# Layjins/Spider

Hardware: AMD Instinct MI355X
Metric: multimodal responses/sec (text->text+image) (higher is better)
Workload: dtype bf16

## Files before the change

### include/spider_hip.h

```cpp
#ifndef SPIDER_HIP_H
#define SPIDER_HIP_H
#define SPIDER_ABI_VERSION 4

#ifdef __cplusplus
extern "C" {
#endif

int spider_abi_version(void);
const char* spider_target_arch(void);
const char* spider_last_error(void);


int spider_embed_bf16(const void* table, const int* ids, void* out, int rows, int H, int V, void* stream);

int spider_rmsnorm_bf16(const void* x, const void* res, const void* w, void* y, void* res_out, int rows, int H,
                        float eps, void* stream);

int spider_gemv_bf16(const void* W, const void* x, void* out, const void* bias, const void* res, const void* norm_w,
                     float eps, int B, int N, int K, void* stream);

int spider_gemv_swiglu_bf16(const void* W_gate_up, const void* x, void* out, const void* norm_w, float eps, int B,
                            int I, int K, void* stream);

int spider_lm_head_nparts(int V);

int spider_decode_advance_i32(const int* next_ids, int* cur_ids, int* pos, int* slot, int* kv_end, int* hist, int* n_hist,
                              int cap, int B, void* stream);
int spider_lm_head_argmax_bf16(const void* W, const void* x, const void* norm_w, float eps, int* out_ids, void* logits,
                               void* ws_val, void* ws_idx, int B, int V, int K, void* stream);

int spider_lm_head_argmax_proc_bf16(const void* W, const void* x, const void* norm_w, float eps, int* out_ids, void* logits,
                                    void* ws_val, void* ws_idx, const void* seen, const void* ban, const float* penalty,
                                    const int* min_new, const int* eos_ids, const int* n_eos, const int* n_hist, int B, int V,
                                    int K, void* stream);
int spider_decode_advance_seen_i32(const int* next_ids, int* cur_ids, int* pos, int* slot, int* kv_end, int* hist, int* n_hist,
                                   void* seen, int V, int cap, int B, void* stream);
int spider_token_bitmap_set_i32(const int* ids, void* bitmap, int B, int n, int V, void* stream);

int spider_beam_partial_bf16(const void* logits, float* ws_ms, float* ws_val, int* ws_tok, int rows, int V, int C, int nslice,
                             void* stream);
int spider_beam_select_f32(const float* ws_ms, const float* ws_val, const int* ws_tok, float* run_scores, const int* eos_ids,
                           const int* n_eos, const int* n_hist, float* trace_score, int* trace_beam, int* trace_tok, int cap,
                           int* src_beam, int* next_ids, int B, int K, int V, int C, int nslice, void* stream);
int spider_kv_row_gather_bf16(void* k_cache, void* v_cache, void* k_tmp, void* v_tmp, const int* src_beam, const int* kv_beg,
                              const int* kv_end, int K, int R, int layers, int rows_alloc, int n_kv, int T, int d, void* stream);

int spider_rope_kv_append_bf16(const void* qkv, const int* pos, const int* slot, const float* cos_sin, void* q_out,
                               void* k_cache, void* v_cache, int B, int S, int n_q, int n_kv, int d, int T_max,
                               void* stream);
int spider_rope_kv_append_mrope_bf16(const void* qkv, const int* pos3, const int* slot, const float* cos_sin, void* q_out,
                                     void* k_cache, void* v_cache, int B, int S, int n_q, int n_kv, int d, int T_max,
                                     int sec_t, int sec_h, void* stream);

int spider_attn_decode_bf16(const void* q, const void* k_cache, const void* v_cache, const int* kv_beg,
                            const int* kv_end, void* out, void* ws_o, void* ws_ml, int B, int n_q, int n_kv, int d,
                            int T_max, float scale, int nsplit, void* stream);

int spider_attn_decode_fused_bf16(const void* qkv, const int* pos, const float* cos_sin, void* k_cache, void* v_cache,
                                  const int* kv_beg, const int* kv_end, void* out, void* ws_o, void* ws_ml,
                                  int* counters, int B, int n_q, int n_kv, int d, int T_max, float scale, int nsplit,
                                  void* stream);
int spider_set_attn_inline(int on);
int spider_set_ws_inlaunch(int on);

int spider_gemv_fm_bf16(const void* Wfm, const void* x, void* out, const void* bias, const void* res, int B, int N, int K,
                        int fold_rmsnorm, float eps, void* stream);
int spider_gemv_swiglu_fm_bf16(const void* Wfm_gate_up, const void* x, void* out, int B, int I, int K, int fold_rmsnorm, float eps,
                               void* stream);
int spider_lm_head_argmax_fm_bf16(const void* Wfm, const void* x, int* out_ids, void* logits, void* ws_val, void* ws_idx, int B,
                                  int V, int K, int fold_rmsnorm, float eps, void* stream);
int spider_lm_head_argmax_fm_proc_bf16(const void* Wfm, const void* x, int* out_ids, void* logits, void* ws_val, void* ws_idx,
                                       const void* seen, const void* ban, const float* penalty, const int* min_new,
                                       const int* eos_ids, const int* n_eos, const int* n_hist, int B, int V, int K,
                                       int fold_rmsnorm, float eps, void* stream);


int spider_gemm_bf16(const void* A, const void* W, void* C, void* C32, const void* bias, const void* res,
                     const void* rowbias, int rows_per_group, int M, int N, int K, int lda, int ldc, int act,
                     float out_scale, int w_tiled, const float* res32, float* c32d, void* ws, long ws_bytes, void* stream);

int spider_gemm_ln_bf16(const void* A, const void* Wf, void* C, const float* colsum, const float* colbias, const void* res,
                        int M, int N, int K, int ldc, int act, float eps, int w_tiled, void* ws, long ws_bytes, void* stream);

int spider_xattn_fused_bf16(const void* x, const void* mq_fm, const void* mo_fm, const float* colsum, const float* colbias,
                            const void* bias_o, void* out, int B2, int n_tok, int C, int heads, int n_keys, float eps,
                            const float* x32, float* out32, void* stream);

int spider_conv2d_nhwc_bf16(const void* x, const void* w, void* y, const void* bias, const void* res,
                            const void* rowbias, int B, int Hin, int Win, int Cin, int Cout, int ks, int stride,
                            int pad, int ups, float out_scale, int w_tiled, const float* res32, float* c32d, void* ws, long ws_bytes, void* stream);

int spider_conv_nhwc_ex_bf16(const void* x, const void* w, void* y, const void* bias, const void* res,
                             const void* rowbias, int B, int Hin, int Win, int Cin, int Cout, int kh, int kw, int stride,
                             int pad_h, int pad_w, int dil, int up_h, int up_w, int act, float act_param,
                             float out_scale, int w_tiled, const float* res32, float* c32d, void* ws, long ws_bytes, void* stream);

int spider_attn_bf16(const void* q, const void* k, const void* v, void* o,
                     long q_bs, long q_hs, long q_rs, long k_bs, long k_hs, long k_rs,
                     long v_bs, long v_hs, long v_rs, long o_bs, long o_hs, long o_rs,
                     int B, int Hq, int Hkv, int Lq, int Lk, int d, float scale, int causal, int kv_off,
                     const int* kv_beg, const void* keep_bits, int blk, int q_off, void* stream);

int spider_story_key_lists_i32(const void* keep_bits, int n_keys, int N, int img0, int n_lists, int q_img0, int stride,
                               int* key_idx, int* tiles, void* stream);
int spider_attn_keylist_bf16(const void* q, const void* k, const void* v, void* o,
                             long q_bs, long q_hs, long q_rs, long k_bs, long k_hs, long k_rs,
                             long v_bs, long v_hs, long v_rs, long o_bs, long o_hs, long o_rs,
                             int B, int Hq, int Hkv, int Lq, int Lk, int d, float scale,
                             const int* key_idx, int idx_len, const int* tiles, int n_tiles, void* stream);

int spider_attn_varlen_bf16(const void* q, const void* k, const void* v, void* o, long q_rs, long k_rs, long v_rs, long o_rs,
                            int total_rows, int Hq, int Hkv, int d, float scale, const int* tiles, int n_tiles, void* stream);

int spider_rope_rows_bf16(void* x, const float* cos_sin, long row_stride, int rows, int heads, int d, void* stream);


int spider_groupnorm_nchunk(int HW);
int spider_groupnorm_nhwc_bf16(const void* x, const void* gamma, const void* beta, void* y, void* ws, int B, int HW,
                               int C, int G, float eps, int silu, void* stream);
int spider_groupnorm_cat_nhwc_bf16(const void* x1, const void* x2, const void* gamma, const void* beta, void* y, void* cat,
                                   void* ws, int B, int HW, int C1, int C2, int G, float eps, int silu, void* stream);
int spider_conv_nhwc_gn_bf16(const void* x, const void* w, void* y, const void* bias, const void* res, const void* rowbias,
                             int B, int Hin, int Win, int Cin, int Cout, int kh, int kw, int stride, int pad_h, int pad_w,
                             int dil, int up_h, int up_w, int act, float act_param, float out_scale, int w_tiled,
                             const float* res32, float* c32d, void* ws, long ws_bytes, void* stream,
                             float* gn_part, int gn_groups, int* produced);
int spider_groupnorm_stats_nhwc_bf16(const void* x, void* partial, int B, int HW, int C, int G, int nchunk, void* stream);
int spider_groupnorm_apply_nhwc_bf16(const void* x, const void* partial, int nchunk, const void* gamma, const void* beta, void* y,
                                     int B, int HW, int C, int G, float eps, int silu, void* stream);
int spider_gemm_gn_in_bf16(const void* A, const void* W, void* C, const void* bias, int M, int N, int K, int ldc, int w_tiled,
                           const float* gn_part, int nchunk, const void* gamma, const void* beta, int G, float eps, int HW,
                           float* c32d, void* stream);
int spider_layernorm_bf16(const void* x, const void* gamma, const void* beta, void* y, int rows, int C, float eps,
                          void* stream);
int spider_geglu_bf16(const void* x, void* y, int M, int inner, void* stream);
int spider_swiglu_bf16(const void* x, void* y, int M, int inner, void* stream);
int spider_concat_channels_bf16(const void* a, const void* b, void* y, long rows, int C1, int C2, void* stream);
int spider_act_bf16(const void* x, void* y, long n, int act, void* stream);
int spider_add_bf16(const void* a, const void* b, void* y, long n, void* stream);
int spider_act_ex_bf16(const void* x, void* y, long n, int act, float param, void* stream);
int spider_add_scaled_bf16(const void* a, const void* b, void* y, long n, float scale, void* stream);
int spider_axpby_bf16(const void* a, const void* b, void* y, long n, float alpha, float beta, void* stream);
int spider_mean_tokens_bf16(const void* x, void* y, int B, int T, int C, void* stream);
int spider_moe_combine_bf16(const void* const* host_xs, int E, const void* logits, int ld, void* y, int B, long per_batch,
                            void* stream);
// ... 132 lines not shown
```

### spider_amd/csrc/llm_decode.hip

```cpp
#include "common.hpp"
#include <stdlib.h>

using namespace spider;

__global__ __launch_bounds__(256) void embed_kernel(const bf16_t* __restrict__ table, const int* __restrict__ ids,
                                                    bf16_t* __restrict__ out, int H, int V) {
    const int r = blockIdx.x;
    int id = ids[r];
    id = id < 0 ? 0 : (id >= V ? V - 1 : id);
    const u32x4* src = reinterpret_cast<const u32x4*>(table + (size_t)id * H);
    u32x4* dst = reinterpret_cast<u32x4*>(out + (size_t)r * H);
    for (int i = threadIdx.x; i < H / 8; i += 256) dst[i] = src[i];
}

__global__ __launch_bounds__(256) void rope_rows_kernel(bf16_t* __restrict__ x, const float* __restrict__ cs, long row_stride,
                                                        int rows, int heads, int d) {
    const int half = d >> 1, cpr = half >> 3;
    const long total = (long)rows * heads * cpr;
    for (long idx = (long)blockIdx.x * 256 + threadIdx.x; idx < total; idx += (long)gridDim.x * 256) {
        const int c = (int)(idx % cpr);
        const int h = (int)((idx / cpr) % heads);
        const long r = idx / ((long)cpr * heads);
        bf16_t* p = x + r * row_stride + (long)h * d + c * 8;
        const u32x4 lo = *reinterpret_cast<const u32x4*>(p);
// ... 13 lines not shown
            float r0 = b0 * co[2 * j], r1 = a0 * si[2 * j], r2 = b1 * co[2 * j + 1], r3 = a1 * si[2 * j + 1];
            asm volatile("" : "+v"(p0), "+v"(p1), "+v"(p2), "+v"(p3), "+v"(r0), "+v"(r1), "+v"(r2), "+v"(r3));
            ol[j] = pack_bf16x2(p0 - p1, p2 - p3);
            oh[j] = pack_bf16x2(r0 + r1, r2 + r3);
        }
        u32x4 vl, vh;
        vl.x = ol[0]; vl.y = ol[1]; vl.z = ol[2]; vl.w = ol[3];
        vh.x = oh[0]; vh.y = oh[1]; vh.z = oh[2]; vh.w = oh[3];
        *reinterpret_cast<u32x4*>(p) = vl;
        *reinterpret_cast<u32x4*>(p + half) = vh;
    }
}

__global__ __launch_bounds__(256) void rmsnorm_kernel(const bf16_t* __restrict__ x, const bf16_t* __restrict__ res,
                                                      const bf16_t* __restrict__ w, bf16_t* __restrict__ y,
                                                      bf16_t* __restrict__ res_out, int H, float eps) {
    __shared__ float red[4];
    const size_t row = blockIdx.x;
    const u32x4* xv = reinterpret_cast<const u32x4*>(x + row * H);
    const u32x4* rv = res ? reinterpret_cast<const u32x4*>(res + row * H) : nullptr;
    const u32x4* wv = reinterpret_cast<const u32x4*>(w);
    u32x4* yv = reinterpret_cast<u32x4*>(y + row * H);
    u32x4* rov = res_out ? reinterpret_cast<u32x4*>(res_out + row * H) : nullptr;
    const int nv = H / 8;
    float h[4][8];
    float ss = 0.f;
#pragma unroll
    for (int it = 0; it < 4; ++it) {
        const int i = threadIdx.x + it * 256;
        if (i < nv) {
            u32x4 a = xv[i];
            uint32_t aw[4] = {a.x, a.y, a.z, a.w};
            if (rv) {
                u32x4 b = rv[i];
                uint32_t bw[4] = {b.x, b.y, b.z, b.w};
#pragma unroll
                for (int j = 0; j < 4; ++j) {
                    float lo = bf16_to_f32(f32_to_bf16(bf16lo_to_f32(aw[j]) + bf16lo_to_f32(bw[j])));
                    float hi = bf16_to_f32(f32_to_bf16(bf16hi_to_f32(aw[j]) + bf16hi_to_f32(bw[j])));
                    h[it][2 * j] = lo;
                    h[it][2 * j + 1] = hi;
                }
                if (rov) {
                    u32x4 o;
                    o.x = pack_bf16x2(h[it][0], h[it][1]);
                    o.y = pack_bf16x2(h[it][2], h[it][3]);
                    o.z = pack_bf16x2(h[it][4], h[it][5]);
                    o.w = pack_bf16x2(h[it][6], h[it][7]);
                    rov[i] = o;
                }
            } else {
#pragma unroll
                for (int j = 0; j < 4; ++j) {
                    h[it][2 * j] = bf16lo_to_f32(aw[j]);
                    h[it][2 * j + 1] = bf16hi_to_f32(aw[j]);
                }
            }
#pragma unroll
            for (int j = 0; j < 8; ++j) ss += h[it][j] * h[it][j];
        }
    }
    const float tot = block_sum<4>(ss, red);
    const float rs = rsqrtf(tot / (float)H + eps);
#pragma unroll
    for (int it = 0; it < 4; ++it) {
        const int i = threadIdx.x + it * 256;
        if (i < nv) {
            u32x4 wq = wv[i];
            uint32_t ww[4] = {wq.x, wq.y, wq.z, wq.w};
            uint32_t o[4];
#pragma unroll
            for (int j = 0; j < 4; ++j) {
                float lo = bf16_to_f32(f32_to_bf16(h[it][2 * j] * rs)) * bf16lo_to_f32(ww[j]);
                float hi = bf16_to_f32(f32_to_bf16(h[it][2 * j + 1] * rs)) * bf16hi_to_f32(ww[j]);
                o[j] = pack_bf16x2(lo, hi);
            }
            u32x4 ov;
            ov.x = o[0]; ov.y = o[1]; ov.z = o[2]; ov.w = o[3];
            yv[i] = ov;
        }
    }
}

template <int NB, int R, bool GATEUP, bool XLDS, int NWB = 4>
__global__ __launch_bounds__(NWB * 64) void gemv_kernel(const bf16_t* __restrict__ W, const bf16_t* __restrict__ x,
                                                   bf16_t* __restrict__ out, const bf16_t* __restrict__ bias,
                                                   const bf16_t* __restrict__ res, const bf16_t* __restrict__ norm_w,
                                                   float eps, int N, int K, int hoist) {
    extern __shared__ __attribute__((aligned(16))) char smem[];
    bf16_t* xs = reinterpret_cast<bf16_t*>(smem);
    __shared__ float red[NWB];
    const int lane = threadIdx.x & 63, wave = threadIdx.x >> 6;
    constexpr int NR = GATEUP ? 2 * R : R;
    constexpr int U = (NR * NB <= 4) ? 4 : 2;

    const int col0 = (blockIdx.x * NWB + wave) * R;
    const bf16_t* wrow[NR];
#pragma unroll
    for (int r = 0; r < R; ++r) {
        int n = col0 + r;
        n = n < N ? n : N - 1;
        wrow[r] = W + (size_t)n * K;
        if (GATEUP) wrow[R + r] = W + (size_t)(N + n) * K;
    }
    u32x4 w0[U][NR];
    if (hoist) {
#pragma unroll
        for (int u = 0; u < U; ++u) {
            const int k = lane * 8 + u * 512;
            if (k < K) {
#pragma unroll
                for (int r = 0; r < NR; ++r)
                    w0[u][r] = __builtin_nontemporal_load(reinterpret_cast<const u32x4*>(wrow[r] + k));
            }
        }
    }

    if (XLDS) {
        const int nv = K / 8;
        for (int b = 0; b < NB; ++b) {
            const u32x4* xv = reinterpret_cast<const u32x4*>(x + (size_t)b * K);
            u32x4* sv = reinterpret_cast<u32x4*>(xs + (size_t)b * K);
            if (norm_w) {
                float ss = 0.f;
                for (int i = threadIdx.x; i < nv; i += NWB * 64) {
                    u32x4 a = xv[i];
                    uint32_t aw[4] = {a.x, a.y, a.z, a.w};
#pragma unroll
                    for (int j = 0; j < 4; ++j) {
                        float lo = bf16lo_to_f32(aw[j]), hi = bf16hi_to_f32(aw[j]);
                        ss += lo * lo + hi * hi;
                    }
                }
                const float rs = rsqrtf(block_sum<NWB>(ss, red) / (float)K + eps);
                const u32x4* wv = reinterpret_cast<const u32x4*>(norm_w);
                for (int i = threadIdx.x; i < nv; i += NWB * 64) {
                    u32x4 a = xv[i], wq = wv[i];
                    uint32_t aw[4] = {a.x, a.y, a.z, a.w}, ww[4] = {wq.x, wq.y, wq.z, wq.w}, o[4];
#pragma unroll
                    for (int j = 0; j < 4; ++j) {
                        float lo = bf16_to_f32(f32_to_bf16(bf16lo_to_f32(aw[j]) * rs)) * bf16lo_to_f32(ww[j]);
                        float hi = bf16_to_f32(f32_to_bf16(bf16hi_to_f32(aw[j]) * rs)) * bf16hi_to_f32(ww[j]);
                        o[j] = pack_bf16x2(lo, hi);
                    }
                    u32x4 ov;
                    ov.x = o[0]; ov.y = o[1]; ov.z = o[2]; ov.w = o[3];
                    sv[i] = ov;
                }
            } else {
                for (int i = threadIdx.x; i < nv; i += NWB * 64) sv[i] = xv[i];
            }
        }
        __syncthreads();
    }

    if (col0 >= N) return;
    float acc[NB][NR];
#pragma unroll
    for (int b = 0; b < NB; ++b)
#pragma unroll
        for (int r = 0; r < NR; ++r) acc[b][r] = 0.f;

    auto fma_w = [&](const u32x4 (&wq)[U][NR], int k0) {
#pragma unroll
        for (int u = 0; u < U; ++u) {
            const int k = k0 + u * 512;
            if (k < K) {
#pragma unroll
                for (int b = 0; b < NB; ++b) {
                    u32x4 xq = XLDS ? *reinterpret_cast<const u32x4*>(xs + (size_t)b * K + k)
                                    : *reinterpret_cast<const u32x4*>(x + (size_t)b * K + k);
                    const uint32_t xw[4] = {xq.x, xq.y, xq.z, xq.w};
#pragma unroll
                    for (int r = 0; r < NR; ++r) {
                        const uint32_t ww[4] = {wq[u][r].x, wq[u][r].y, wq[u][r].z, wq[u][r].w};
#pragma unroll
                        for (int j = 0; j < 4; ++j) acc[b][r] = dot2_bf16(ww[j], xw[j], acc[b][r]);
                    }
                }
            }
        }
    };
    int kstart = lane * 8;
    if (hoist) {
        fma_w(w0, kstart);
        kstart += 512 * U;
    }
    for (int k0 = kstart; k0 < K; k0 += 512 * U) {
        u32x4 wq[U][NR];
#pragma unroll
        for (int u = 0; u < U; ++u) {
            const int k = k0 + u * 512;
            if (k < K) {
#pragma unroll
                for (int r = 0; r < NR; ++r)
                    wq[u][r] = __builtin_nontemporal_load(reinterpret_cast<const u32x4*>(wrow[r] + k));
            }
        }
        fma_w(wq, k0);
    }
#pragma unroll
    for (int b = 0; b < NB; ++b)
#pragma unroll
        for (int r = 0; r < NR; ++r) acc[b][r] = wave_sum(acc[b][r]);

    if (lane == 0) {
#pragma unroll
        for (int r = 0; r < R; ++r) {
            const int n = col0 + r;
            if (n < N) {
#pragma unroll
                for (int b = 0; b < NB; ++b) {
                    float v;
                    if (GATEUP) {
                        const float g = bf16_to_f32(f32_to_bf16(acc[b][r]));
                        const float u = bf16_to_f32(f32_to_bf16(acc[b][R + r]));
                        const float a = bf16_to_f32(f32_to_bf16(silu_f(g)));
                        v = a * u;
                    } else {
                        v = acc[b][r];
                        if (bias) v += bf16_to_f32(bias[n]);
                        if (res) v = bf16_to_f32(f32_to_bf16(v)) + bf16_to_f32(res[(size_t)b * N + n]);
                    }
                    out[(size_t)b * N + n] = f32_to_bf16(v);
                }
            }
        }
    }
}

struct LmProc {
    const uint32_t* seen;
    const uint32_t* ban;
    const float* penalty;
    const int* min_new;
    const int* eos_ids;
    const int* n_eos;
    const int* n_hist;
    int words;
};

__device__ __forceinline__ uint32_t lm_proc_flags(const LmProc& pr, int b, int n) {
    const size_t w = (size_t)b * pr.words + (n >> 5);
    const uint32_t bit = 1u << (n & 31);
    uint32_t f = (pr.seen[w] & bit) ? 1u : 0u;
    if (pr.ban[w] & bit) f |= 2u;
    if (pr.n_hist[b] < pr.min_new[0]) {
        const int ne = min(pr.n_eos[0], 8);
        for (int e = 0; e < ne; ++e)
            if (pr.eos_ids[e] == n) f |= 2u;
    }
    return f;
}

__device__ __forceinline__ float lm_proc_apply(float lv, uint32_t flags, float p) {
    if (flags & 1u) lv = lv < 0.f ? lv * p : __fdiv_rn(lv, p);
    if (flags & 2u) lv = -INFINITY;
    return lv;
}

template <int NB, int R, bool PROC = false>
__global__ __launch_bounds__(256) void lmhead_partial_kernel(const bf16_t* __restrict__ W, const bf16_t* __restrict__ x,
                                                             const bf16_t* __restrict__ norm_w, float eps,
                                                             float* __restrict__ pval, int* __restrict__ pidx,
                                                             bf16_t* __restrict__ logits, int V, int K, LmProc pr) {
    extern __shared__ __attribute__((aligned(16))) char smem[];
    bf16_t* xs = reinterpret_cast<bf16_t*>(smem);
    __shared__ float red[4];
    __shared__ float bval[4][NB];
    __shared__ int bidx[4][NB];
    const int lane = threadIdx.x & 63, wave = threadIdx.x >> 6;
    const int nv = K / 8;
    for (int b = 0; b < NB; ++b) {
        const u32x4* xv = reinterpret_cast<const u32x4*>(x + (size_t)b * K);
        u32x4* sv = reinterpret_cast<u32x4*>(xs + (size_t)b * K);
        if (norm_w) {
            float ss = 0.f;
            for (int i = threadIdx.x; i < nv; i += 256) {
                u32x4 a = xv[i];
                uint32_t aw[4] = {a.x, a.y, a.z, a.w};
#pragma unroll
                for (int j = 0; j < 4; ++j) {
// ... 815 lines not shown
#pragma unroll
                for (int w = 0; w < NW; ++w) tot += ssq[w][r16];
                rs = rsqrtf(tot / (float)K + eps);
            }
#pragma unroll
            for (int t = 0; t < TN; ++t)
#pragma unroll
                for (int j = 0; j < 4; ++j) {
                    float a = 0.f;
#pragma unroll
                    for (int w = 0; w < NW; ++w) a += part[w][t][lane][j];
                    v[t][j] = a * rs;
                }
            const int m = r16;
            if (MODE == 2) {
                float lb = -INFINITY;
                int li = 0x7fffffff;
                uint32_t sw = 0, bw = 0;
                float pen = 1.f;
                bool no_eos = false;
                if (PROC) {
                    const int nn0 = 16 * rg + 4 * g;
                    if (nn0 < N && m < B) {
                        const size_t w = (size_t)m * pr.words + (nn0 >> 5);
                        sw = pr.seen[w] >> (nn0 & 31);
                        bw = pr.ban[w] >> (nn0 & 31);
                        no_eos = pr.n_hist[m] < pr.min_new[0];
                    }
                    pen = pr.penalty[0];
                }
#pragma unroll
                for (int j = 0; j < 4; ++j) {
                    const int nn = 16 * rg + 4 * g + j;
                    const bf16_t q = f32_to_bf16(v[0][j]);
                    float lv = bf16_to_f32(q);
                    if (nn < N && m < B) {
                        if (out) out[(size_t)m * N + nn] = q;
                        if (PROC) {
                            uint32_t fl = ((sw >> j) & 1u) | (((bw >> j) & 1u) << 1);
                            if (no_eos) {
                                const int ne = min(pr.n_eos[0], 8);
                                for (int e = 0; e < ne; ++e)
                                    if (pr.eos_ids[e] == nn) fl |= 2u;
                            }
                            lv = lm_proc_apply(lv, fl, pen);
                            if (lv > lb || (lv == lb && nn < li)) { lb = lv; li = nn; }
                        } else if (lv > lb) { lb = lv; li = nn; }
                    }
                }
#pragma unroll
                for (int off = 16; off <= 32; off <<= 1) {
                    const float ov = __shfl_xor(lb, off, 64);
                    const int oi = __shfl_xor(li, off, 64);
                    if (ov > lb || (ov == lb && oi < li)) { lb = ov; li = oi; }
                }
                if (lb > best || (lb == best && li < besti)) { best = lb; besti = li; }
            } else if (m < B) {
#pragma unroll
                for (int j = 0; j < 4; ++j) {
                    const int nn = 16 * rg + 4 * g + j;
                    if (nn < N) {
                        float o;
                        if (GATEUP) {
                            const float gg = bf16_to_f32(f32_to_bf16(v[0][j])), uu = bf16_to_f32(f32_to_bf16(v[TN - 1][j]));
                            o = bf16_to_f32(f32_to_bf16(silu_f(gg))) * uu;
                        } else {
                            o = v[0][j];
                            if (bias) o += bf16_to_f32(bias[nn]);
                            if (res) o = bf16_to_f32(f32_to_bf16(o)) + bf16_to_f32(res[(size_t)m * N + nn]);
                        }
                        out[(size_t)m * N + nn] = f32_to_bf16(o);
                    }
                }
            }
        }
        if (MODE == 2) __syncthreads();
    }
    if (MODE == 2 && wave == 0 && lane < 16 && lane < B) {
        pval[(size_t)lane * gridDim.x + blockIdx.x] = best;
        pidx[(size_t)lane * gridDim.x + blockIdx.x] = besti;
    }
}

#define GEMV_ARGS (const bf16_t*)W, (const bf16_t*)x, (bf16_t*)out, (const bf16_t*)bias, (const bf16_t*)res, (const bf16_t*)norm_w, eps, N, K, hoist
#define GEMV_LAUNCH(NB_, R_, GU_, XL_)                                                                         \
    do {                                                                                                        \
        if (wide8) gemv_kernel<NB_, R_, GU_, XL_, 8><<<(N + 8 * R_ - 1) / (8 * R_), 512, XL_ ? (size_t)NB_ * K * 2 : 0, (hipStream_t)stream>>>(GEMV_ARGS); \
        else gemv_kernel<NB_, R_, GU_, XL_, 4><<<grid, 256, XL_ ? (size_t)NB_ * K * 2 : 0, (hipStream_t)stream>>>(GEMV_ARGS); \
    } while (0)

static int gemv_env_r() {
    static const int v = [] { const char* e = getenv("SPIDER_GEMV_R"); return e ? atoi(e) : 0; }();
    return v;
}

template <int NB, bool GU>
static int gemv_dispatch(const void* W, const void* x, void* out, const void* bias, const void* res,
                         const void* norm_w, float eps, int N, int K, void* stream) {
    static const size_t xlds_max = [] { const char* e = getenv("SPIDER_GEMV_XLDS_MAX"); return e ? (size_t)atol(e) : (size_t)64 * 1024; }();
    const bool xlds = (size_t)NB * K * 2 <= xlds_max || norm_w != nullptr;
    if (!xlds) SPIDER_CHECK(norm_w == nullptr, "gemv: fused RMSNorm needs batch*K*2 <= 64 KiB");
    SPIDER_CHECK((size_t)NB * K * 2 <= 64 * 1024 || norm_w == nullptr, "gemv: fused RMSNorm needs batch*K*2 <= 64 KiB");
    static const int hoist = [] { const char* e = getenv("SPIDER_GEMV_HOIST"); return e ? atoi(e) : 1; }();
    int R = GU ? 1 : 2;
    if (!GU && (size_t)N * K * 2 < (size_t)48 << 20) R = 1;
    if (gemv_env_r()) R = gemv_env_r();
    if (GU && R > 2) R = 2;
    if (NB > 4 && R > 2) R = 2;
    const int grid = (N + 4 * R - 1) / (4 * R);
    static const int wide_env = [] { const char* e = getenv("SPIDER_GEMV_WIDE8"); return e ? atoi(e) : -1; }();
    const bool wide8 = wide_env >= 0 ? wide_env != 0 : (!GU && K >= 8192 && NB == 1);
#define GEMV_PICK(R_)                                   \
    do {                                                \
        if (xlds) GEMV_LAUNCH(NB, R_, GU, true);        \
        else GEMV_LAUNCH(NB, R_, GU, false);            \
    } while (0)
    if (R == 1) GEMV_PICK(1);
    else if (R == 2) GEMV_PICK(2);
    else GEMV_PICK(4);
#undef GEMV_PICK
    SPIDER_LAUNCH_OK();
    return 0;
}

template <bool GU>
static int gemv_batch(const void* W, const void* x, void* out, const void* bias, const void* res, const void* norm_w,
                      float eps, int B, int N, int K, void* stream) {
    static const int mfma_min_b = [] { const char* e = getenv("SPIDER_GEMV_MFMA_MIN_B"); return e ? atoi(e) : 5; }();
    if (B >= mfma_min_b && B <= 16 && K % 64 == 0 && norm_w == nullptr) {
        skinny_gemm_kernel<GU, 8><<<(N + 15) / 16, 512, 0, (hipStream_t)stream>>>((const bf16_t*)W, (const bf16_t*)x, (bf16_t*)out,
                                                                                  (const bf16_t*)bias, (const bf16_t*)res, B, N, K);
        SPIDER_LAUNCH_OK();
        return 0;
    }
    switch (B) {
        case 1: return gemv_dispatch<1, GU>(W, x, out, bias, res, norm_w, eps, N, K, stream);
        case 2: return gemv_dispatch<2, GU>(W, x, out, bias, res, norm_w, eps, N, K, stream);
        case 3: return gemv_dispatch<3, GU>(W, x, out, bias, res, norm_w, eps, N, K, stream);
        case 4: return gemv_dispatch<4, GU>(W, x, out, bias, res, norm_w, eps, N, K, stream);
        case 5: return gemv_dispatch<5, GU>(W, x, out, bias, res, norm_w, eps, N, K, stream);
        case 6: return gemv_dispatch<6, GU>(W, x, out, bias, res, norm_w, eps, N, K, stream);
        case 7: return gemv_dispatch<7, GU>(W, x, out, bias, res, norm_w, eps, N, K, stream);
        case 8: return gemv_dispatch<8, GU>(W, x, out, bias, res, norm_w, eps, N, K, stream);
        default: spider_set_error("gemv: batch must be 1..8 (1..16 when K % 64 == 0 and norm_w == NULL; use spider_gemm_bf16 beyond that)"); return -1;
    }
}


#define SPIDER_ATTN_INLINE_DEFAULT 0
static int g_attn_inline = -1;

extern "C" {

int spider_set_attn_inline(int on) {
    const int prev = g_attn_inline;
    g_attn_inline = on < 0 ? 0 : (on > 2 ? 2 : on);
    return prev;
}

int spider_embed_bf16(const void* table, const int* ids, void* out, int rows, int H, int V, void* stream) {
    SPIDER_CHECK(rows > 0 && H > 0 && H % 8 == 0 && V > 0, "embed: bad shape (H must be a multiple of 8)");
    embed_kernel<<<rows, 256, 0, (hipStream_t)stream>>>((const bf16_t*)table, ids, (bf16_t*)out, H, V);
    SPIDER_LAUNCH_OK();
    return 0;
}

int spider_rope_rows_bf16(void* x, const float* cos_sin, long row_stride, int rows, int heads, int d, void* stream) {
    SPIDER_CHECK(rows > 0 && heads > 0 && d > 0 && d % 16 == 0, "rope_rows: head_dim must be a multiple of 16");
    SPIDER_CHECK(row_stride % 8 == 0 && row_stride >= (long)heads * d, "rope_rows: row stride must be >= heads*d and keep 16-byte alignment");
    const long total = (long)rows * heads * (d / 16);
    long g = (total + 255) / 256;
    if (g > 8192) g = 8192;
    rope_rows_kernel<<<(int)g, 256, 0, (hipStream_t)stream>>>((bf16_t*)x, cos_sin, row_stride, rows, heads, d);
    SPIDER_LAUNCH_OK();
    return 0;
}

int spider_rmsnorm_bf16(const void* x, const void* res, const void* w, void* y, void* res_out, int rows, int H,
                        float eps, void* stream) {
    SPIDER_CHECK(rows > 0 && H > 0 && H % 8 == 0 && H <= 8192, "rmsnorm: H must be a multiple of 8 and <= 8192");
    rmsnorm_kernel<<<rows, 256, 0, (hipStream_t)stream>>>((const bf16_t*)x, (const bf16_t*)res, (const bf16_t*)w,
                                                          (bf16_t*)y, (bf16_t*)res_out, H, eps);
    SPIDER_LAUNCH_OK();
    return 0;
}

int spider_gemv_bf16(const void* W, const void* x, void* out, const void* bias, const void* res, const void* norm_w,
                     float eps, int B, int N, int K, void* stream) {
    SPIDER_CHECK(N > 0 && K > 0 && K % 8 == 0, "gemv: K must be a positive multiple of 8");
    return gemv_batch<false>(W, x, out, bias, res, norm_w, eps, B, N, K, stream);
}

int spider_gemv_swiglu_bf16(const void* W_gate_up, const void* x, void* out, const void* norm_w, float eps, int B,
                            int I, int K, void* stream) {
    SPIDER_CHECK(I > 0 && K > 0 && K % 8 == 0, "gemv_swiglu: K must be a positive multiple of 8");
    return gemv_batch<true>(W_gate_up, x, out, nullptr, nullptr, norm_w, eps, B, I, K, stream);
}

#define LMHEAD_LAUNCH(NB_)                                                                                     \
    lmhead_partial_kernel<NB_, 2><<<nparts, 256, (size_t)NB_ * K * 2, (hipStream_t)stream>>>(                   \
        (const bf16_t*)W, (const bf16_t*)x, (const bf16_t*)norm_w, eps, (float*)ws_val, (int*)ws_idx,          \
        (bf16_t*)logits, V, K, LmProc{})
#define LMHEAD_PROC_LAUNCH(NB_)                                                                                \
    lmhead_partial_kernel<NB_, 2, true><<<nparts, 256, (size_t)NB_ * K * 2, (hipStream_t)stream>>>(             \
        (const bf16_t*)W, (const bf16_t*)x, (const bf16_t*)norm_w, eps, (float*)ws_val, (int*)ws_idx,          \
        (bf16_t*)logits, V, K, pr)

int spider_decode_advance_i32(const int* next_ids, int* cur_ids, int* pos, int* slot, int* kv_end, int* hist, int* n_hist,
                              int cap, int B, void* stream) {
    SPIDER_CHECK(next_ids && cur_ids && pos && slot && kv_end && B > 0, "decode_advance: cursors required");
    SPIDER_CHECK(!hist || (n_hist && cap > 0), "decode_advance: history needs its counters and capacity");
    decode_advance_kernel<<<(B + 63) / 64, 64, 0, (hipStream_t)stream>>>(next_ids, cur_ids, pos, slot, kv_end, hist, n_hist, cap, B);
    SPIDER_LAUNCH_OK();
    return 0;
}

int spider_decode_advance_seen_i32(const int* next_ids, int* cur_ids, int* pos, int* slot, int* kv_end, int* hist, int* n_hist,
                                   void* seen, int V, int cap, int B, void* stream) {
    SPIDER_CHECK(next_ids && cur_ids && pos && slot && kv_end && B > 0, "decode_advance_seen: cursors required");
    SPIDER_CHECK(!hist || (n_hist && cap > 0), "decode_advance_seen: history needs its counters and capacity");
    SPIDER_CHECK(seen && V > 0, "decode_advance_seen: bitmap and vocabulary size required");
    decode_advance_seen_kernel<<<(B + 63) / 64, 64, 0, (hipStream_t)stream>>>(next_ids, cur_ids, pos, slot, kv_end, hist, n_hist,
                                                                            (uint32_t*)seen, V, cap, B);
    SPIDER_LAUNCH_OK();
    return 0;
}

int spider_token_bitmap_set_i32(const int* ids, void* bitmap, int B, int n, int V, void* stream) {
    SPIDER_CHECK(ids && bitmap && B > 0 && n > 0 && V > 0, "token_bitmap_set: ids [B, n], bitmap and V > 0 required");
    const long total = (long)B * n;
    token_bitmap_set_kernel<<<(unsigned)((total + 255) / 256), 256, 0, (hipStream_t)stream>>>(ids, (uint32_t*)bitmap, B, n, V);
    SPIDER_LAUNCH_OK();
    return 0;
}

// ... 228 lines not shown
```

### spider_amd/lib.py

```python
from __future__ import annotations

import ctypes as C
import os
import threading

import torch

_HERE = os.path.dirname(os.path.abspath(__file__))
LIB_PATH = os.path.join(_HERE, "libspider_hip.so")

_lib = None
_lock = threading.Lock()

_vp, _i, _f, _l = C.c_void_p, C.c_int, C.c_float, C.c_long

SIGNATURES = {
    "spider_abi_version": (_i, []),
    "spider_target_arch": (C.c_char_p, []),
    "spider_last_error": (C.c_char_p, []),
    "spider_embed_bf16": (_i, [_vp, _vp, _vp, _i, _i, _i, _vp]),
    "spider_rmsnorm_bf16": (_i, [_vp, _vp, _vp, _vp, _vp, _i, _i, _f, _vp]),
    "spider_gemv_bf16": (_i, [_vp, _vp, _vp, _vp, _vp, _vp, _f, _i, _i, _i, _vp]),
    "spider_gemv_swiglu_bf16": (_i, [_vp, _vp, _vp, _vp, _f, _i, _i, _i, _vp]),
    "spider_lm_head_nparts": (_i, [_i]),
    "spider_decode_advance_i32": (_i, [_vp] * 7 + [_i, _i, _vp]),
    "spider_lm_head_argmax_bf16": (_i, [_vp, _vp, _vp, _f, _vp, _vp, _vp, _vp, _i, _i, _i, _vp]),
    "spider_lm_head_argmax_proc_bf16": (_i, [_vp, _vp, _vp, _f] + [_vp] * 11 + [_i, _i, _i, _vp]),
    "spider_decode_advance_seen_i32": (_i, [_vp] * 8 + [_i, _i, _i, _vp]),
    "spider_token_bitmap_set_i32": (_i, [_vp, _vp, _i, _i, _i, _vp]),
    "spider_beam_partial_bf16": (_i, [_vp] * 4 + [_i] * 4 + [_vp]),
    "spider_beam_select_f32": (_i, [_vp] * 10 + [_i, _vp, _vp] + [_i] * 5 + [_vp]),
    "spider_kv_row_gather_bf16": (_i, [_vp] * 7 + [_i] * 7 + [_vp]),
    "spider_gemv_fm_bf16": (_i, [_vp, _vp, _vp, _vp, _vp, _i, _i, _i, _i, _f, _vp]),
    "spider_gemv_swiglu_fm_bf16": (_i, [_vp, _vp, _vp, _i, _i, _i, _i, _f, _vp]),
    "spider_lm_head_argmax_fm_bf16": (_i, [_vp, _vp, _vp, _vp, _vp, _vp, _i, _i, _i, _i, _f, _vp]),
    "spider_lm_head_argmax_fm_proc_bf16": (_i, [_vp] * 13 + [_i, _i, _i, _i, _f, _vp]),
    "spider_rope_kv_append_bf16": (_i, [_vp, _vp, _vp, _vp, _vp, _vp, _vp, _i, _i, _i, _i, _i, _i, _vp]),
    "spider_rope_kv_append_mrope_bf16": (_i, [_vp, _vp, _vp, _vp, _vp, _vp, _vp, _i, _i, _i, _i, _i, _i, _i, _i, _vp]),
    "spider_attn_decode_bf16": (_i, [_vp, _vp, _vp, _vp, _vp, _vp, _vp, _vp, _i, _i, _i, _i, _i, _f, _i, _vp]),
    "spider_attn_decode_fused_bf16": (_i, [_vp] * 11 + [_i, _i, _i, _i, _i, _f, _i, _vp]),
    "spider_set_attn_inline": (_i, [_i]),
    "spider_set_ws_inlaunch": (_i, [_i]),
    "spider_gemm_bf16": (_i, [_vp, _vp, _vp, _vp, _vp, _vp, _vp, _i, _i, _i, _i, _i, _i, _i, _f, _i, _vp, _vp, _vp, _l, _vp]),
    "spider_gemm_ln_bf16": (_i, [_vp, _vp, _vp, _vp, _vp, _vp, _i, _i, _i, _i, _i, _f, _i, _vp, _l, _vp]),
    "spider_xattn_fused_bf16": (_i, [_vp, _vp, _vp, _vp, _vp, _vp, _vp, _i, _i, _i, _i, _i, _f, _vp, _vp, _vp]),
    "spider_conv2d_nhwc_bf16": (_i, [_vp, _vp, _vp, _vp, _vp, _vp, _i, _i, _i, _i, _i, _i, _i, _i, _i, _f, _i, _vp, _vp, _vp, _l, _vp]),
    "spider_conv_nhwc_ex_bf16": (_i, [_vp] * 6 + [_i] * 14 + [_f, _f, _i, _vp, _vp, _vp, _l, _vp]),
    "spider_attn_bf16": (_i, [_vp, _vp, _vp, _vp] + [_l] * 12 + [_i] * 6 + [_f, _i, _i, _vp, _vp, _i, _i, _vp]),
    "spider_story_key_lists_i32": (_i, [_vp, _i, _i, _i, _i, _i, _i, _vp, _vp, _vp]),
    "spider_attn_keylist_bf16": (_i, [_vp, _vp, _vp, _vp] + [_l] * 12 + [_i] * 6 + [_f, _vp, _i, _vp, _i, _vp]),
    "spider_attn_varlen_bf16": (_i, [_vp, _vp, _vp, _vp, _l, _l, _l, _l, _i, _i, _i, _i, _f, _vp, _i, _vp]),
    "spider_rope_rows_bf16": (_i, [_vp, _vp, _l, _i, _i, _i, _vp]),
    "spider_groupnorm_nchunk": (_i, [_i]),
    "spider_groupnorm_nhwc_bf16": (_i, [_vp, _vp, _vp, _vp, _vp, _i, _i, _i, _i, _f, _i, _vp]),
    "spider_groupnorm_cat_nhwc_bf16": (_i, [_vp] * 7 + [_i, _i, _i, _i, _i, _f, _i, _vp]),
    "spider_conv_nhwc_gn_bf16": (_i, [_vp] * 6 + [_i] * 14 + [_f, _f, _i, _vp, _vp, _vp, _l, _vp] + [_vp, _i, _vp]),
    "spider_groupnorm_stats_nhwc_bf16": (_i, [_vp, _vp, _i, _i, _i, _i, _i, _vp]),
    "spider_groupnorm_apply_nhwc_bf16": (_i, [_vp, _vp, _i, _vp, _vp, _vp, _i, _i, _i, _i, _f, _i, _vp]),
    "spider_gemm_gn_in_bf16": (_i, [_vp, _vp, _vp, _vp, _i, _i, _i, _i, _i, _vp, _i, _vp, _vp, _i, _f, _i, _vp, _vp]),
    "spider_layernorm_bf16": (_i, [_vp, _vp, _vp, _vp, _i, _i, _f, _vp]),
    "spider_geglu_bf16": (_i, [_vp, _vp, _i, _i, _vp]),
    "spider_swiglu_bf16": (_i, [_vp, _vp, _i, _i, _vp]),
    "spider_concat_channels_bf16": (_i, [_vp, _vp, _vp, _l, _i, _i, _vp]),
    "spider_act_bf16": (_i, [_vp, _vp, _l, _i, _vp]),
    "spider_add_bf16": (_i, [_vp, _vp, _vp, _l, _vp]),
    "spider_act_ex_bf16": (_i, [_vp, _vp, _l, _i, _f, _vp]),
    "spider_add_scaled_bf16": (_i, [_vp, _vp, _vp, _l, _f, _vp]),
    "spider_axpby_bf16": (_i, [_vp, _vp, _vp, _l, _f, _f, _vp]),
    "spider_mean_tokens_bf16": (_i, [_vp, _vp, _i, _i, _i, _vp]),
    "spider_moe_combine_bf16": (_i, [_vp, _i, _vp, _i, _vp, _i, _l, _vp]),
    "spider_col2im1d_f32_bf16": (_i, [_vp, _vp, _vp, _i, _i, _i, _i, _i, _i, _vp]),
    "spider_l2_normalize_rows_bf16": (_i, [_vp, _vp, _i, _i, _f, _vp]),
    "spider_conv2d_small_cin_bf16": (_i, [_vp, _vp, _vp, _vp, _i, _i, _i, _i, _i, _i, _vp]),
    "spider_conv2d_small_cout_bf16": (_i, [_vp, _vp, _vp, _vp, _vp, _i, _i, _i, _i, _i, _i, _vp]),
    "spider_latent_to_nhwc_bf16": (_i, [_vp, _vp, _i, _i, _i, _i, _f, _vp]),
    "spider_cfg_combine_f32": (_i, [_vp, _vp, _i, _i, _i, _f, _vp]),
    "spider_lincomb_f32": (_i, [_vp, _vp, _i, _vp, _l, _vp]),
    "spider_softmax_rows_f32_bf16": (_i, [_vp, _vp, _i, _i, _i, _f, _vp]),
    "spider_pack_keep_bits_f32": (_i, [_vp, _vp, _i, _i, _f, _vp]),
    "spider_nhwc_to_nchw_f32": (_i, [_vp, _vp, _i, _i, _i, _f, _f, _i, _vp]),
    "spider_gemm_a32_bf16": (_i, [_vp] * 5 + [_i] * 5 + [_f, _i, _vp, _vp, _vp, _l, _vp]),
    "spider_gemm_ln_a32_bf16": (_i, [_vp] * 6 + [_i, _i, _i, _i, _i, _f, _i, _vp]),
    "spider_gemm_gn_in_a32_bf16": (_i, [_vp, _vp, _vp, _vp, _i, _i, _i, _i, _i, _vp, _i, _vp, _vp, _i, _f, _i, _vp, _vp]),
    "spider_conv_nhwc_a32_bf16": (_i, [_vp] * 6 + [_i] * 13 + [_f, _i, _vp, _vp, _vp, _l, _vp]),
    "spider_groupnorm_f32in_nhwc_bf16": (_i, [_vp, _vp, _i, _vp, _vp, _vp, _vp, _vp, _i, _i, _i, _i, _f, _i, _vp]),
    "spider_split_hilo_f32_bf16": (_i, [_vp, _vp, _vp, _l, _vp]),
    "spider_row_split_f32_bf16": (_i, [_vp, _vp, _vp, _vp, _l, _i, _f, _vp]),
    "spider_groupnorm_f32in_split_nhwc_bf16": (_i, [_vp, _vp, _i, _vp, _vp, _vp, _vp, _i, _i, _i, _i, _f, _i, _vp]),
    "spider_conv2d_small_cin_f32in_bf16": (_i, [_vp] * 5 + [_i] * 6 + [_vp]),
    "spider_conv2d_small_cout_f32in_bf16": (_i, [_vp] * 4 + [_i] * 6 + [_vp]),
    "spider_latent_to_nhwc_f32": (_i, [_vp, _vp, _i, _i, _i, _i, _f, _vp]),
}

F16_OPS = (
    "spider_gemm", "spider_gemm_ln", "spider_xattn_fused", "spider_conv2d_nhwc", "spider_conv_nhwc_ex", "spider_attn",
    "spider_conv_nhwc_gn", "spider_groupnorm_stats_nhwc", "spider_groupnorm_apply_nhwc", "spider_gemm_gn_in",
    "spider_attn_keylist", "spider_attn_varlen", "spider_groupnorm_nhwc", "spider_groupnorm_cat_nhwc", "spider_layernorm",
    "spider_geglu", "spider_swiglu", "spider_concat_channels", "spider_act", "spider_add", "spider_act_ex", "spider_add_scaled",
    "spider_axpby", "spider_mean_tokens", "spider_moe_combine", "spider_col2im1d_f32", "spider_l2_normalize_rows",
    "spider_conv2d_small_cin", "spider_conv2d_small_cout", "spider_latent_to_nhwc", "spider_softmax_rows_f32",
    "spider_gemm_a32", "spider_gemm_ln_a32", "spider_gemm_gn_in_a32", "spider_conv_nhwc_a32", "spider_groupnorm_f32in_nhwc", "spider_conv2d_small_cin_f32in",
    "spider_conv2d_small_cout_f32in", "spider_split_hilo_f32", "spider_row_split_f32", "spider_groupnorm_f32in_split_nhwc",
)
for _n in F16_OPS:
    SIGNATURES[_n + "_f16"] = SIGNATURES[_n + "_bf16"]


class SpiderHipError(RuntimeError):
    pass


def load():
    global _lib
    if _lib is not None:
        return _lib
    with _lock:
        if _lib is not None:
            return _lib
        if not os.path.exists(LIB_PATH):
            raise SpiderHipError(
                f"{LIB_PATH} is missing: the HIP extension has not been built "
                "(run `python -c 'import __graft_entry__ as g; g.build()'`). There is no fallback path."
            )
        lib = C.CDLL(LIB_PATH)
# ... 17 lines not shown
```

Before: 1.952.

## Add scheduled GEMV variants overlapping weight prefetch with x staging and double-buffered loads

Adds SCHED template variants to the decode GEMV kernel, on by default with an env/API toggle. The x/norm staging into LDS is batched into register stages and interleaved with the hoisted weight loads. For K<=4096 single-row cases the whole row is hoisted (8 chunks), and for wide8 kernels a double-buffered weight load loop with sched barriers is used. Branchless clamped addressing replaces bounds checks. This aims to hide memory latency in bandwidth-bound decode GEMVs, at the cost of higher register pressure and possibly lower occupancy.

```diff
diff --git a/include/spider_hip.h b/include/spider_hip.h
--- a/include/spider_hip.h
+++ b/include/spider_hip.h
@@ -61,6 +61,7 @@
                                   int* counters, int B, int n_q, int n_kv, int d, int T_max, float scale, int nsplit,
                                   void* stream);
 int spider_set_attn_inline(int on);
+int spider_set_gemv_sched(int sched);
 int spider_set_ws_inlaunch(int on);
 
 int spider_gemv_fm_bf16(const void* Wfm, const void* x, void* out, const void* bias, const void* res, int B, int N, int K,
diff --git a/spider_amd/csrc/llm_decode.hip b/spider_amd/csrc/llm_decode.hip
--- a/spider_amd/csrc/llm_decode.hip
+++ b/spider_amd/csrc/llm_decode.hip
@@ -119,7 +119,9 @@
     }
 }
 
-template <int NB, int R, bool GATEUP, bool XLDS, int NWB = 4>
+constexpr int GEMV_STAGE_CAP(int nwb) { return nwb == 8 ? 6 : 4; }
+
+template <int NB, int R, bool GATEUP, bool XLDS, int NWB = 4, int SCHED = 0>
 __global__ __launch_bounds__(NWB * 64) void gemv_kernel(const bf16_t* __restrict__ W, const bf16_t* __restrict__ x,
                                                    bf16_t* __restrict__ out, const bf16_t* __restrict__ bias,
                                                    const bf16_t* __restrict__ res, const bf16_t* __restrict__ norm_w,
@@ -127,7 +129,7 @@
     extern __shared__ __attribute__((aligned(16))) char smem[];
     bf16_t* xs = reinterpret_cast<bf16_t*>(smem);
     __shared__ float red[NWB];
-    const int lane = threadIdx.x & 63, wave = threadIdx.x >> 6;
+    const int lane = threadIdx.x & 63, wave = SCHED ? __builtin_amdgcn_readfirstlane(threadIdx.x >> 6) : threadIdx.x >> 6;
     constexpr int NR = GATEUP ? 2 * R : R;
     constexpr int U = (NR * NB <= 4) ? 4 : 2;
 
@@ -140,55 +142,156 @@
         wrow[r] = W + (size_t)n * K;
         if (GATEUP) wrow[R + r] = W + (size_t)(N + n) * K;
     }
-    u32x4 w0[U][NR];
-    if (hoist) {
-#pragma unroll
-        for (int u = 0; u < U; ++u) {
-            const int k = lane * 8 + u * 512;
-            if (k < K) {
-#pragma unroll
-                for (int r = 0; r < NR; ++r)
-                    w0[u][r] = __builtin_nontemporal_load(reinterpret_cast<const u32x4*>(wrow[r] + k));
-            }
-        }
-    }
-
-    if (XLDS) {
-        const int nv = K / 8;
-        for (int b = 0; b < NB; ++b) {
-            const u32x4* xv = reinterpret_cast<const u32x4*>(x + (size_t)b * K);
-            u32x4* sv = reinterpret_cast<u32x4*>(xs + (size_t)b * K);
-            if (norm_w) {
-                float ss = 0.f;
-                for (int i = threadIdx.x; i < nv; i += NWB * 64) {
-                    u32x4 a = xv[i];
-                    uint32_t aw[4] = {a.x, a.y, a.z, a.w};
+    constexpr int H = SCHED == 1 ? 8 : U;
+    u32x4 w0[H][NR];
+    if constexpr (SCHED == 0) {
+        if (hoist) {
+#pragma unroll
+            for (int u = 0; u < U; ++u) {
+                const int k = lane * 8 + u * 512;
+                if (k < K) {
+#pragma unroll
+                    for (int r = 0; r < NR; ++r)
+                        w0[u][r] = __builtin_nontemporal_load(reinterpret_cast<const u32x4*>(wrow[r] + k));
+                }
+            }
+        }
+
+        if (XLDS) {
+            const int nv = K / 8;
+            for (int b = 0; b < NB; ++b) {
+                const u32x4* xv = reinterpret_cast<const u32x4*>(x + (size_t)b * K);
+                u32x4* sv = reinterpret_cast<u32x4*>(xs + (size_t)b * K);
+                if (norm_w) {
+                    float ss = 0.f;
+                    for (int i = threadIdx.x; i < nv; i += NWB * 64) {
+                        u32x4 a = xv[i];
+                        uint32_t aw[4] = {a.x, a.y, a.z, a.w};
+#pragma unroll
+                        for (int j = 0; j < 4; ++j) {
+                            float lo = bf16lo_to_f32(aw[j]), hi = bf16hi_to_f32(aw[j]);
+                            ss += lo * lo + hi * hi;
+                        }
+                    }
+                    const float rs = rsqrtf(block_sum<NWB>(ss, red) / (float)K + eps);
+                    const u32x4* wv = reinterpret_cast<const u32x4*>(norm_w);
+                    for (int i = threadIdx.x; i < nv; i += NWB * 64) {
+                        u32x4 a = xv[i], wq = wv[i];
+                        uint32_t aw[4] = {a.x, a.y, a.z, a.w}, ww[4] = {wq.x, wq.y, wq.z, wq.w}, o[4];
+#pragma unroll
+                        for (int j = 0; j < 4; ++j) {
+                            float lo = bf16_to_f32(f32_to_bf16(bf16lo_to_f32(aw[j]) * rs)) * bf16lo_to_f32(ww[j]);
+                            float hi = bf16_to_f32(f32_to_bf16(bf16hi_to_f32(aw[j]) * rs)) * bf16hi_to_f32(ww[j]);
+                            o[j] = pack_bf16x2(lo, hi);
+                        }
+                        u32x4 ov;
+                        ov.x = o[0]; ov.y = o[1]; ov.z = o[2]; ov.w = o[3];
+                        sv[i] = ov;
+                    }
+                } else {
+                    for (int i = threadIdx.x; i < nv; i += NWB * 64) sv[i] = xv[i];
+                }
+            }
+            __syncthreads();
+        }
+
+    } else {
+        constexpr int NT = NWB * 64, CAP = GEMV_STAGE_CAP(NWB), CH = CAP / 2;
+        const int nv = K / 8, t0 = threadIdx.x;
+        const u32x4* wv = reinterpret_cast<const u32x4*>(norm_w);
+        u32x4 st[CAP];
+        auto issue_x = [&](const u32x4* xv, int i0) {
+#pragma unroll
+            for (int c = 0; c < CAP; ++c) st[c] = xv[min(i0 + c * NT, nv - 1)];
+        };
+        auto issue_xw = [&](const u32x4* xv, int i0) {
+#pragma unroll
+            for (int c = 0; c < CH; ++c) st[c] = xv[min(i0 + c * NT, nv - 1)];
+#pragma unroll
+            for (int c = 0; c < CH; ++c) st[CH + c] = wv[min(i0 + c * NT, nv - 1)];
+        };
+        auto store_x = [&](u32x4* sv, int i0) {
+#pragma unroll
+            for (int c = 0; c < CAP; ++c) sv[min(i0 + c * NT, nv - 1)] = st[c];
+        };
+        auto sumsq = [&](float ss, int i0, int n) {
+#pragma unroll
+            for (int c = 0; c < CAP; ++c) {
+                if (c < n) {
+                    const bool in = i0 + c * NT < nv;
+                    uint32_t aw[4] = {in ? st[c].x : 0u, in ? st[c].y : 0u, in ? st[c].z : 0u, in ? st[c].w : 0u};
 #pragma unroll
                     for (int j = 0; j < 4; ++j) {
                         float lo = bf16lo_to_f32(aw[j]), hi = bf16hi_to_f32(aw[j]);
                         ss += lo * lo + hi * hi;
                     }
                 }
+            }
+            return ss;
+        };
+        auto norm_store = [&](u32x4* sv, int i0, float rs) {
+#pragma unroll
+            for (int c = 0; c < CH; ++c) {
+                const u32x4 a = st[c], wq = st[CH + c];
+                uint32_t aw[4] = {a.x, a.y, a.z, a.w}, ww[4] = {wq.x, wq.y, wq.z, wq.w}, o[4];
+#pragma unroll
+                for (int j = 0; j < 4; ++j) {
+                    float lo = bf16_to_f32(f32_to_bf16(bf16lo_to_f32(aw[j]) * rs)) * bf16lo_to_f32(ww[j]);
+                    float hi = bf16_to_f32(f32_to_bf16(bf16hi_to_f32(aw[j]) * rs)) * bf16hi_to_f32(ww[j]);
+                    o[j] = pack_bf16x2(lo, hi);
+                }
+                u32x4 ov;
+                ov.x = o[0]; ov.y = o[1]; ov.z = o[2]; ov.w = o[3];
+                sv[min(i0 + c * NT, nv - 1)] = ov;
+            }
+        };
+        auto hoist_w = [&]() {
+#pragma unroll
+            for (int u = 0; u < H; ++u) {
+                const int k = lane * 8 + u * 512;
+#pragma unroll
+                for (int r = 0; r < NR; ++r)
+                    w0[u][r] = __builtin_nontemporal_load(reinterpret_cast<const u32x4*>(wrow[r] + (unsigned)(k < K ? k : K - 8)));
+            }
+        };
+        const u32x4* xv = reinterpret_cast<const u32x4*>(x);
+        u32x4* sv = reinterpret_cast<u32x4*>(xs);
+        if (!XLDS) {
+            hoist_w();
+        } else if (!norm_w) {
+            issue_x(xv, t0);
+            hoist_w();
+            store_x(sv, t0);
+            asm volatile("" ::: "memory");
+            for (int b = 0; b < NB; ++b)
+                for (int i0 = b ? 0 : CAP * NT; i0 < nv; i0 += CAP * NT) {
+                    issue_x(xv + (size_t)b * nv, i0 + t0);
+                    store_x(sv + (size_t)b * nv, i0 + t0);
+                }
+        } else if (nv <= CH * NT) {
+            issue_xw(xv, t0);
+            hoist_w();
+            for (int b = 0; b < NB; ++b) {
+                if (b) issue_xw(xv + (size_t)b * nv, t0);
+                const float rs = rsqrtf(block_sum<NWB>(sumsq(0.f, t0, CH), red) / (float)K + eps);
+                norm_store(sv + (size_t)b * nv, t0, rs);
+            }
+        } else {
+            hoist_w();
+            for (int b = 0; b < NB; ++b) {
+                float ss = 0.f;
+                for (int i0 = 0; i0 < nv; i0 += CAP * NT) {
+                    issue_x(xv + (size_t)b * nv, i0 + t0);
+                    ss = sumsq(ss, i0 + t0, CAP);
+                }
                 const float rs = rsqrtf(block_sum<NWB>(ss, red) / (float)K + eps);
-                const u32x4* wv = reinterpret_cast<const u32x4*>(norm_w);
-                for (int i = threadIdx.x; i < nv; i += NWB * 64) {
-                    u32x4 a = xv[i], wq = wv[i];
-                    uint32_t aw[4] = {a.x, a.y, a.z, a.w}, ww[4] = {wq.x, wq.y, wq.z, wq.w}, o[4];
-#pragma unroll
-                    for (int j = 0; j < 4; ++j) {
-                        float lo = bf16_to_f32(f32_to_bf16(bf16lo_to_f32(aw[j]) * rs)) * bf16lo_to_f32(ww[j]);
-                        float hi = bf16_to_f32(f32_to_bf16(bf16hi_to_f32(aw[j]) * rs)) * bf16hi_to_f32(ww[j]);
-                        o[j] = pack_bf16x2(lo, hi);
-                    }
-                    u32x4 ov;
-                    ov.x = o[0]; ov.y = o[1]; ov.z = o[2]; ov.w = o[3];
-                    sv[i] = ov;
-                }
-            } else {
-                for (int i = threadIdx.x; i < nv; i += NWB * 64) sv[i] = xv[i];
-            }
-        }
-        __syncthreads();
+                for (int i0 = 0; i0 < nv; i0 += CH * NT) {
+                    issue_xw(xv + (size_t)b * nv, i0 + t0);
+                    norm_store(sv + (size_t)b * nv, i0 + t0, rs);
+                }
+            }
+        }
+        if (XLDS) __syncthreads();
     }
 
     if (col0 >= N) return;
@@ -218,23 +321,97 @@
             }
         }
     };
-    int kstart = lane * 8;
-    if (hoist) {
-        fma_w(w0, kstart);
-        kstart += 512 * U;
-    }
-    for (int k0 = kstart; k0 < K; k0 += 512 * U) {
-        u32x4 wq[U][NR];
-#pragma unroll
-        for (int u = 0; u < U; ++u) {
-            const int k = k0 + u * 512;
-            if (k < K) {
+    auto fma_chunk = [&](const u32x4 (&wq)[NR], int k, bool full) {
+        if (full || k < K) {
+#pragma unroll
+            for (int b = 0; b < NB; ++b) {
+                u32x4 xq = XLDS ? *reinterpret_cast<const u32x4*>(xs + (size_t)b * K + k)
+                                : *reinterpret_cast<const u32x4*>(x + (size_t)b * K + k);
+                const uint32_t xw[4] = {xq.x, xq.y, xq.z, xq.w};
+#pragma unroll
+                for (int r = 0; r < NR; ++r) {
+                    const uint32_t ww[4] = {wq[r].x, wq[r].y, wq[r].z, wq[r].w};
+#pragma unroll
+                    for (int j = 0; j < 4; ++j) acc[b][r] = dot2_bf16(ww[j], xw[j], acc[b][r]);
+                }
+            }
+        }
+    };
+    if constexpr (SCHED == 1) {
+#pragma unroll
+        for (int u = 0; u < H; ++u) fma_chunk(w0[u], lane * 8 + u * 512, false);
+    } else if constexpr (SCHED == 2 && NWB == 8) {
+        constexpr int S = 512 * U;
+        u32x4 w1[U][NR];
+        auto load_set = [&](u32x4 (&wq)[U][NR], int base) {
+#pragma unroll
+            for (int u = 0; u < U; ++u) {
+                const int k = base + lane * 8 + u * 512;
 #pragma unroll
                 for (int r = 0; r < NR; ++r)
-                    wq[u][r] = __builtin_nontemporal_load(reinterpret_cast<const u32x4*>(wrow[r] + k));
-            }
-        }
-        fma_w(wq, k0);
+                    wq[u][r] = __builtin_nontemporal_load(reinterpret_cast<const u32x4*>(wrow[r] + (unsigned)(k < K ? k : K - 8)));
+            }
+        };
+        auto fma_set = [&](const u32x4 (&wq)[U][NR], int base, bool full) {
+#pragma unroll
+            for (int u = 0; u < U; ++u) fma_chunk(wq[u], base + lane * 8 + u * 512, full);
+        };
+        const int nfull = (K - 1) / S;
+        if (nfull == 0) {
+            fma_set(w0, 0, false);
+        } else {
+            load_set(w1, S);
+            fma_set(w0, 0, true);
+            int s = 1;
+            for (; s + 2 <= nfull; s += 2) {
+                __builtin_amdgcn_sched_barrier(0);
+                load_set(w0, (s + 1) * S);
+                fma_set(w1, s * S, true);
+                __builtin_amdgcn_sched_barrier(0);
+                load_set(w1, (s + 2) * S);
+                fma_set(w0, (s + 1) * S, true);
+            }
+            __builtin_amdgcn_sched_barrier(0);
+            if (s < nfull) {
+                load_set(w0, (s + 1) * S);
+                fma_set(w1, s * S, true);
+                fma_set(w0, (s + 1) * S, false);
+            } else {
+                fma_set(w1, s * S, false);
+            }
+        }
+    } else if constexpr (SCHED == 2) {
+        fma_w(w0, lane * 8);
+        for (int k0 = lane * 8 + 512 * U; k0 < K; k0 += 512 * U) {
+            u32x4 wq[U][NR];
+#pragma unroll
+            for (int u = 0; u < U; ++u) {
+                const int k = k0 + u * 512;
+#pragma unroll
+                for (int r = 0; r < NR; ++r)
+                    wq[u][r] = __builtin_nontemporal_load(reinterpret_cast<const u32x4*>(wrow[r] + (unsigned)(k < K ? k : K - 8)));
+            }
+            fma_w(wq, k0);
+        }
+    } else {
+        int kstart = lane * 8;
+        if (hoist) {
+            fma_w(w0, kstart);
+            kstart += 512 * U;
+        }
+        for (int k0 = kstart; k0 < K; k0 += 512 * U) {
+            u32x4 wq[U][NR];
+#pragma unroll
+            for (int u = 0; u < U; ++u) {
+                const int k = k0 + u * 512;
+                if (k < K) {
+#pragma unroll
+                    for (int r = 0; r < NR; ++r)
+                        wq[u][r] = __builtin_nontemporal_load(reinterpret_cast<const u32x4*>(wrow[r] + k));
+                }
+            }
+            fma_w(wq, k0);
+        }
     }
 #pragma unroll
     for (int b = 0; b < NB; ++b)
@@ -1216,11 +1393,24 @@
     }
 }
 
+static int g_gemv_sched = -1;
+static int gemv_sched() {
+    if (g_gemv_sched < 0) { const char* e = getenv("SPIDER_GEMV_SCHED"); g_gemv_sched = e ? (atoi(e) != 0) : 1; }
+    return g_gemv_sched;
+}
+
 #define GEMV_ARGS (const bf16_t*)W, (const bf16_t*)x, (bf16_t*)out, (const bf16_t*)bias, (const bf16_t*)res, (const bf16_t*)norm_w, eps, N, K, hoist
 #define GEMV_LAUNCH(NB_, R_, GU_, XL_)                                                                         \
     do {                                                                                                        \
-        if (wide8) gemv_kernel<NB_, R_, GU_, XL_, 8><<<(N + 8 * R_ - 1) / (8 * R_), 512, XL_ ? (size_t)NB_ * K * 2 : 0, (hipStream_t)stream>>>(GEMV_ARGS); \
-        else gemv_kernel<NB_, R_, GU_, XL_, 4><<<grid, 256, XL_ ? (size_t)NB_ * K * 2 : 0, (hipStream_t)stream>>>(GEMV_ARGS); \
+        const size_t lds_ = XL_ ? (size_t)NB_ * K * 2 : 0;                                                      \
+        constexpr bool ROW_ = !GU_ && R_ * NB_ <= 2 && XL_;                                                   \
+        if (wide8) {                                                                                            \
+            if (sched) gemv_kernel<NB_, R_, GU_, XL_, 8, 2><<<(N + 8 * R_ - 1) / (8 * R_), 512, lds_, (hipStream_t)stream>>>(GEMV_ARGS); \
+            else gemv_kernel<NB_, R_, GU_, XL_, 8><<<(N + 8 * R_ - 1) / (8 * R_), 512, lds_, (hipStream_t)stream>>>(GEMV_ARGS); \
+        } else if (sched == 1 && ROW_) {                                                                        \
+            if constexpr (ROW_) gemv_kernel<NB_, R_, GU_, XL_, 4, 1><<<grid, 256, lds_, (hipStream_t)stream>>>(GEMV_ARGS); \
+        } else if (sched) gemv_kernel<NB_, R_, GU_, XL_, 4, 2><<<grid, 256, lds_, (hipStream_t)stream>>>(GEMV_ARGS); \
+        else gemv_kernel<NB_, R_, GU_, XL_, 4><<<grid, 256, lds_, (hipStream_t)stream>>>(GEMV_ARGS);            \
     } while (0)
 
 static int gemv_env_r() {
@@ -1244,6 +1434,7 @@
     const int grid = (N + 4 * R - 1) / (4 * R);
     static const int wide_env = [] { const char* e = getenv("SPIDER_GEMV_WIDE8"); return e ? atoi(e) : -1; }();
     const bool wide8 = wide_env >= 0 ? wide_env != 0 : (!GU && K >= 8192 && NB == 1);
+    const int sched = !(hoist && gemv_sched()) ? 0 : (K <= 4096 ? 1 : 2);
 #define GEMV_PICK(R_)                                   \
     do {                                                \
         if (xlds) GEMV_LAUNCH(NB, R_, GU, true);        \
@@ -1285,6 +1476,12 @@
 static int g_attn_inline = -1;
 
 extern "C" {
+
+int spider_set_gemv_sched(int sched) {
+    const int prev = gemv_sched();
+    g_gemv_sched = sched != 0;
+    return prev;
+}
 
 int spider_set_attn_inline(int on) {
     const int prev = g_attn_inline;
diff --git a/spider_amd/lib.py b/spider_amd/lib.py
--- a/spider_amd/lib.py
+++ b/spider_amd/lib.py
@@ -40,6 +40,7 @@
     "spider_attn_decode_bf16": (_i, [_vp, _vp, _vp, _vp, _vp, _vp, _vp, _vp, _i, _i, _i, _i, _i, _f, _i, _vp]),
     "spider_attn_decode_fused_bf16": (_i, [_vp] * 11 + [_i, _i, _i, _i, _i, _f, _i, _vp]),
     "spider_set_attn_inline": (_i, [_i]),
+    "spider_set_gemv_sched": (_i, [_i]),
     "spider_set_ws_inlaunch": (_i, [_i]),
     "spider_gemm_bf16": (_i, [_vp, _vp, _vp, _vp, _vp, _vp, _vp, _i, _i, _i, _i, _i, _i, _i, _f, _i, _vp, _vp, _vp, _l, _vp]),
     "spider_gemm_ln_bf16": (_i, [_vp, _vp, _vp, _vp, _vp, _vp, _i, _i, _i, _i, _i, _f, _i, _vp, _l, _vp]),
```

After: 2.013 (median of 6 runs). 1.03x the previous value.
